# achiever04/face-recognition-platform

Hardware: AMD Instinct MI355X
Metric: faces/sec (detect+embed+match) on 1080p @ 100k gallery (higher is better)
Workload: dtype f16; 1 GPU; 32x1080x1920 BGR frames per GPU per step resident in HBM, host results out every step, 2 batches in flight per GPU (one handle = one stream each, used round-robin), forced K=10 faces/frame, 100000-identity fp16 gallery, FRPDet detector fp16 + ArcFace IResNet-100 fp16 (synthetic seeded weights); batch_frames=32, faces_per_frame=10, gallery=100000, streams=1, lanes=2, lane_warmup_steps=20

## Files before the change

face-recognition-platform_amd/csrc/stem_kernel.hip:

```cpp
#include <hip/hip_runtime.h>
#include <stdint.h>
#include "frp_internal.h"
#include "conv_common.h"

namespace frp {


#define ST_ROWS 4
#define ST_COLS 64
#define ST_PR (2 * ST_ROWS + 1)
#define ST_PE ((2 * ST_COLS + 1) * 3)
#define ST_PITCH 392

__device__ __forceinline__ void bias_relu_pack(const floatx16& acc, int g, floatx4 b, unsigned (&out)[2]) {
#pragma unroll
    for (int h2 = 0; h2 < 2; ++h2) {
        const float2v v = float2v{acc[4 * g + 2 * h2], acc[4 * g + 2 * h2 + 1]} + float2v{b[2 * h2], b[2 * h2 + 1]};
        half2v hv = __builtin_convertvector(v, half2v);
        hv = __builtin_elementwise_max(hv, half2v{0, 0});
        out[h2] = __builtin_bit_cast(unsigned, hv);
    }
}

__device__ __forceinline__ floatx16 mfma16(half8 a, half8 b, floatx16 c) {
    return __builtin_amdgcn_mfma_f32_32x32x16_f16(a, b, c, 0, 0, 0);
}

__global__ __launch_bounds__(256) void stem_u8_kernel(StemParams p) {
    __shared__ __attribute__((aligned(16))) _Float16 patch[ST_PR * ST_PITCH + 16];
    const int t = threadIdx.x, lane = t & 63, wave = t >> 6;
    const int tiles_x = (p.Wo + ST_COLS - 1) / ST_COLS;
    const int tiles_y = (p.Ho + ST_ROWS - 1) / ST_ROWS;
    int bid = blockIdx.x;
    const int tx = bid % tiles_x; bid /= tiles_x;
    const int ty = bid % tiles_y;
    const int b = bid / tiles_y;
    const int oy0 = ty * ST_ROWS, ox0 = tx * ST_COLS;
    const uint8_t* frame = p.frames + (long)b * p.frame_stride;

    const int ix_first = 2 * ox0 - 1;
#pragma unroll
    for (int pr = 0; pr < ST_PR; ++pr) {
        const int iy = 2 * oy0 - 1 + pr;
        const bool yin = (unsigned)iy < (unsigned)p.Hc;
        const bool yimg = (unsigned)iy < (unsigned)p.H;
        const uint8_t* row = frame + (long)(yimg ? iy : 0) * p.row_stride;
        for (int e = t; e < ST_PE; e += 256) {
            const int px = e / 3;
            const int ix = ix_first + px;
            float v = 0.f;
            if (yin && (unsigned)ix < (unsigned)p.Wc) {
                float u = 0.f;
                if (yimg && ix < p.W) u = (float)row[(long)ix * 3 + (e - px * 3)];
                v = (u - 127.5f) * (1.0f / 128.0f);
            }
            const int c = e - px * 3;
            patch[pr * ST_PITCH + px * 3 + (p.rgb_in ? c : 2 - c)] = (_Float16)v;
        }
    }
    for (int e = t; e < ST_PR * (ST_PITCH - ST_PE) + 16; e += 256) {
        if (e < ST_PR * (ST_PITCH - ST_PE)) {
            const int pr = e / (ST_PITCH - ST_PE), off = e - pr * (ST_PITCH - ST_PE);
            patch[pr * ST_PITCH + ST_PE + off] = (_Float16)0.f;
        } else {
            patch[ST_PR * ST_PITCH + (e - ST_PR * (ST_PITCH - ST_PE))] = (_Float16)0.f;
        }
    }

    half8 wa[3];
    {
        const int co = lane & 31, h = lane >> 5;
#pragma unroll
        for (int kh = 0; kh < 3; ++kh)
#pragma unroll
            for (int j = 0; j < 8; ++j) {
                const int k = 8 * h + j;
                _Float16 w = (_Float16)0.f;
                if (k < 9) {
                    const int kw = k / 3, c = k - kw * 3;
                    w = p.w[((co * 3 + kh) * 3 + kw) * 8 + c];
                }
                wa[kh][j] = w;
            }
    }
    __syncthreads();

    const int oy = oy0 + wave;
    const int r = lane & 31, h = lane >> 5;
    const floatx4 bias4[4] = {*reinterpret_cast<const floatx4*>(p.bias + 4 * h), *reinterpret_cast<const floatx4*>(p.bias + 8 + 4 * h),
                              *reinterpret_cast<const floatx4*>(p.bias + 16 + 4 * h), *reinterpret_cast<const floatx4*>(p.bias + 24 + 4 * h)};
#pragma unroll
    for (int half_tile = 0; half_tile < ST_COLS / 32; ++half_tile) {
        const int oxl = half_tile * 32 + r;
        const unsigned* win = reinterpret_cast<const unsigned*>(patch + (2 * wave) * ST_PITCH + 6 * oxl + 8 * h);
        floatx16 acc;
#pragma unroll
        for (int e = 0; e < 16; ++e) acc[e] = 0.f;
#pragma unroll
        for (int kh = 0; kh < 3; ++kh) {
            union { unsigned u[4]; half8 v; } bf;
#pragma unroll
            for (int q = 0; q < 4; ++q) bf.u[q] = win[kh * (ST_PITCH / 2) + q];
            acc = mfma16(wa[kh], bf.v, acc);
        }
        const int ox = ox0 + oxl;
        union { half4 v; unsigned u[2]; } pk[4];
#pragma unroll
        for (int g = 0; g < 4; ++g)
#pragma unroll
            for (int e = 0; e < 4; ++e) pk[g].v[e] = (_Float16)fmaxf(acc[4 * g + e] + bias4[g][e], 0.f);
#pragma unroll
        for (int q = 0; q < 2; ++q) {
            swap_halves(pk[2 * q].u[0], pk[2 * q + 1].u[0]);
            swap_halves(pk[2 * q].u[1], pk[2 * q + 1].u[1]);
        }
        if (oy < p.Ho && ox < p.Wo) {
            _Float16* o = p.out + (((long)b * p.Ho + oy) * p.Wo + ox) * 32;
#pragma unroll
            for (int q = 0; q < 2; ++q)
                *reinterpret_cast<uint4*>(o + 16 * q + 8 * h) = make_uint4(pk[2 * q].u[0], pk[2 * q].u[1], pk[2 * q + 1].u[0], pk[2 * q + 1].u[1]);
        }
    }
}

#define S12_R2 4
#define S12_C2 32
#define S12_S1R (2 * S12_R2 + 1)
#define S12_S1C (2 * S12_C2 + 1)
#define S12_PR (2 * S12_S1R + 1)
#define S12_PE ((2 * S12_S1C + 1) * 3)
#define S12_PITCH 400
#define S12_PATCH_HALFS (S12_PR * S12_PITCH + 16)
#define S12_PIX 80
#define S12_S1BYTES (S12_S1R * 2 * 33 * S12_PIX)

__global__ __launch_bounds__(256, 2) void stem12_u8_kernel(Stem12Params p) {
    __shared__ __attribute__((aligned(16))) _Float16 patch[S12_PATCH_HALFS];
    __shared__ __attribute__((aligned(16))) unsigned char s1[S12_S1BYTES];
    const int t = threadIdx.x, lane = t & 63, wave = t >> 6;
    const int r = lane & 31, h = lane >> 5;
    const int tiles_x = (p.Wo2 + S12_C2 - 1) / S12_C2;
    const int tiles_y = (p.Ho2 + S12_R2 - 1) / S12_R2;
    const int n_tiles = p.B * tiles_y * tiles_x;

    half8 wa[3];
    {
        const int co = r;
#pragma unroll
        for (int kh = 0; kh < 3; ++kh)
#pragma unroll
            for (int j = 0; j < 8; ++j) {
                const int k = 8 * h + j;
                _Float16 w = (_Float16)0.f;
                if (k < 9) {
                    const int kw = k / 3, c = k - kw * 3;
                    w = p.w1[((co * 3 + kh) * 3 + kw) * 8 + 2 - c];
                }
                wa[kh][j] = w;
            }
    }
    const int g2 = wave & 1;
    half8 wb[18];
#pragma unroll
    for (int m = 0; m < 18; ++m)
        wb[m] = *reinterpret_cast<const half8*>(p.w2 + (((g2 * 32 + r) * 9 + (m >> 1)) * 32 + 16 * (m & 1) + 8 * h));
    floatx4 b1[4], b2[4];
#pragma unroll
    for (int g = 0; g < 4; ++g) {
        b1[g] = *reinterpret_cast<const floatx4*>(p.bias1 + 8 * g + 4 * h);
        b2[g] = *reinterpret_cast<const floatx4*>(p.bias2 + 32 * g2 + 8 * g + 4 * h);
    }
    for (int e = t; e < S12_PATCH_HALFS; e += 256) patch[e] = (_Float16)0.f;
    __syncthreads();

    constexpr int DW_ROW = 99;
    constexpr int DW_PER_THREAD = (S12_PR * DW_ROW + 255) / 256;
    const uint8_t* const buf_lo = p.frames;
    const uint8_t* const buf_hi = p.frames + (long)p.B * p.frame_stride;
    unsigned pre[DW_PER_THREAD];
    int rel[DW_PER_THREAD], ldso[DW_PER_THREAD];
#pragma unroll
    for (int i = 0; i < DW_PER_THREAD; ++i) {
        const int idx = t + i * 256;
        const int pr = idx / DW_ROW, d = idx - pr * DW_ROW;
        rel[i] = pr < S12_PR ? pr * (int)p.row_stride + 4 * d : -1;
        ldso[i] = (pr * S12_PITCH + 4 * d) * 2;
    }
    bool pre_fast = false;
    auto tile_interior = [&](int y2_0, int x2_0) {
        const int iy0 = 4 * y2_0 - 3, ix0 = 4 * x2_0 - 3;
        return iy0 >= 0 && iy0 + S12_PR <= p.H && ix0 >= 0 && ix0 + (2 * S12_S1C + 1) + 1 <= p.W;
    };
    auto tile_coords = [&](int tile, int& b, int& y2_0, int& x2_0) {
        int q = tile;
        const int tx = q % tiles_x; q /= tiles_x;
        const int ty = q % tiles_y;
        b = q / tiles_y;
        y2_0 = ty * S12_R2;
        x2_0 = tx * S12_C2;
    };
    auto row_addr = [&](int b, int y2_0, int x2_0, int pr) -> const uint8_t* {
        int iy = 4 * y2_0 - 3 + pr;
        iy = iy < 0 ? 0 : (iy >= p.H ? p.H - 1 : iy);
        return p.frames + (long)b * p.frame_stride + (long)iy * p.row_stride + (long)(4 * x2_0 - 3) * 3;
    };
    auto prefetch = [&](int tile) {
        int b, y2_0, x2_0;
        tile_coords(tile, b, y2_0, x2_0);
        pre_fast = !p.rgb_in && tile_interior(y2_0, x2_0);
        if (pre_fast) {
            const uint8_t* base = p.frames + (long)b * p.frame_stride + (long)(4 * y2_0 - 3) * p.row_stride + (long)(4 * x2_0 - 3) * 3;
#pragma unroll
            for (int i = 0; i < DW_PER_THREAD; ++i) {
                unsigned v = 0u;
                if (rel[i] >= 0) __builtin_memcpy(&v, base + (unsigned)rel[i], 4);
                pre[i] = v;
            }
            return;
        }
#pragma unroll
        for (int i = 0; i < DW_PER_THREAD; ++i) {
            const int idx = t + i * 256;
            const int pr = idx / DW_ROW, d = idx - pr * DW_ROW;
            unsigned v = 0u;
            if (pr < S12_PR) {
                const uint8_t* a = row_addr(b, y2_0, x2_0, pr);
                const uint8_t* al = a - ((uintptr_t)a & 3) + 4 * d;
                if (al >= buf_lo && al + 4 <= buf_hi) {
                    v = *reinterpret_cast<const unsigned*>(al);
                } else {
#pragma unroll
                    for (int j = 0; j < 4; ++j)
                        if (al + j >= buf_lo && al + j < buf_hi) v |= (unsigned)al[j] << (8 * j);
                }
            }
            pre[i] = v;
        }
    };
    if ((int)blockIdx.x < n_tiles) prefetch(blockIdx.x);

    for (int tile = blockIdx.x; tile < n_tiles; tile += gridDim.x) {
        int b, y2_0, x2_0;
        tile_coords(tile, b, y2_0, x2_0);
        const int s1r0 = 2 * y2_0 - 1, s1c0 = 2 * x2_0 - 1;
        const int iy0 = 2 * s1r0 - 1, ix0 = 2 * s1c0 - 1;

        const bool interior = iy0 >= 0 && iy0 + S12_PR <= p.H && ix0 >= 0 && ix0 + (2 * S12_S1C + 1) <= p.W;
        if (pre_fast) {
            const half2v k1024 = {(_Float16)1024.f, (_Float16)1024.f}, kscale = {(_Float16)0.0078125f, (_Float16)0.0078125f},
                         kbias = {(_Float16)-0.99609375f, (_Float16)-0.99609375f};
#pragma unroll
            for (int i = 0; i < DW_PER_THREAD; ++i) {
                if (rel[i] >= 0) {
                    const unsigned lo = __builtin_amdgcn_perm(0x64646464u, pre[i], 0x04010400u);
                    const unsigned hi = __builtin_amdgcn_perm(0x64646464u, pre[i], 0x04030402u);
                    const half2v a = __builtin_elementwise_fma(__builtin_bit_cast(half2v, lo) - k1024, kscale, kbias);
                    const half2v c = __builtin_elementwise_fma(__builtin_bit_cast(half2v, hi) - k1024, kscale, kbias);
                    *reinterpret_cast<uint2*>(reinterpret_cast<unsigned char*>(patch) + ldso[i]) =
                        make_uint2(__builtin_bit_cast(unsigned, a), __builtin_bit_cast(unsigned, c));
                }
            }
        } else {
#pragma unroll
        for (int i = 0; i < DW_PER_THREAD; ++i) {
            const int idx = t + i * 256;
            const int pr = idx / DW_ROW, d = idx - pr * DW_ROW;
            if (pr < S12_PR) {
                const int sh = (int)((uintptr_t)row_addr(b, y2_0, x2_0, pr) & 3);
                const int e0 = 4 * d - sh;
                int px = (e0 + 3) / 3 - 1, c = e0 - px * 3;
                _Float16* prow = patch + pr * S12_PITCH;
                const int iy = iy0 + pr;
                const bool yin = (unsigned)iy < (unsigned)p.Hc;
                const bool yimg = (unsigned)iy < (unsigned)p.H;
#pragma unroll
                for (int j = 0; j < 4; ++j) {
                    const int e = e0 + j;
                    if (e >= 0 && e < S12_PE) {
                        float v = ((float)((pre[i] >> (8 * j)) & 0xffu) - 127.5f) * (1.0f / 128.0f);
                        if (!interior) {
                            const int ix = ix0 + px;
                            const bool in_canvas = yin && (unsigned)ix < (unsigned)p.Wc;
                            const bool in_frame = yimg && ix < p.W;
                            v = in_canvas ? (in_frame ? v : (0.f - 127.5f) * (1.0f / 128.0f)) : 0.f;
                        }
                        prow[px * 3 + (p.rgb_in ? 2 - c : c)] = (_Float16)v;
                    }
                    if (++c == 3) { c = 0; ++px; }
                }
            }
        }
        for (int e = t; e < S12_PR * (S12_PITCH - S12_PE); e += 256) {
            const int pr = e / (S12_PITCH - S12_PE);
            patch[pr * S12_PITCH + S12_PE + (e - pr * (S12_PITCH - S12_PE))] = (_Float16)0.f;
        }
        }
        __syncthreads();
        if (tile + (int)gridDim.x < n_tiles) prefetch(tile + gridDim.x);

        for (int job = wave; job < S12_S1R * 2 + 1; job += 4) {
            const bool extra = job == S12_S1R * 2;
            const int row = extra ? (r < S12_S1R ? r : 0) : job >> 1;
            const int col = extra ? 2 * S12_C2 : (job & 1) * 32 + r;
            const unsigned* win = reinterpret_cast<const unsigned*>(patch + (2 * row) * S12_PITCH + 6 * col + 8 * h);
            floatx16 acc;
#pragma unroll
            for (int e = 0; e < 16; ++e) acc[e] = 0.f;
#pragma unroll
            for (int kh = 0; kh < 3; ++kh) {
                union { unsigned u[4]; half8 v; } bf;
#pragma unroll
                for (int qq = 0; qq < 4; ++qq) bf.u[qq] = win[kh * (S12_PITCH / 2) + qq];
                acc = mfma16(wa[kh], bf.v, acc);
            }
            const int gy = s1r0 + row, gx = s1c0 + col;
            const bool inside = (unsigned)gy < (unsigned)p.Ho1 && (unsigned)gx < (unsigned)p.Wo1;
            struct { unsigned u[2]; } pk[4];
#pragma unroll
            for (int g = 0; g < 4; ++g) {
                bias_relu_pack(acc, g, b1[g], pk[g].u);
                pk[g].u[0] = inside ? pk[g].u[0] : 0u;
                pk[g].u[1] = inside ? pk[g].u[1] : 0u;
            }
#pragma unroll
            for (int qq = 0; qq < 2; ++qq) {
                swap_halves(pk[2 * qq].u[0], pk[2 * qq + 1].u[0]);
                swap_halves(pk[2 * qq].u[1], pk[2 * qq + 1].u[1]);
            }
            if (!extra || r < S12_S1R) {
                unsigned char* dst = s1 + ((row * 2 + (col & 1)) * 33 + (col >> 1)) * S12_PIX;
#pragma unroll
                for (int qq = 0; qq < 2; ++qq)
                    *reinterpret_cast<uint4*>(dst + (2 * qq + h) * 16) =
                        make_uint4(pk[2 * qq].u[0], pk[2 * qq].u[1], pk[2 * qq + 1].u[0], pk[2 * qq + 1].u[1]);
            }
        }
        __syncthreads();

#pragma unroll
        for (int yy = 0; yy < 2; ++yy) {
            const int y = 2 * (wave >> 1) + yy;
            floatx16 acc;
#pragma unroll
            for (int e = 0; e < 16; ++e) acc[e] = 0.f;
#pragma unroll
            for (int m = 0; m < 18; ++m) {
                const int tap = m >> 1, kh = tap / 3, kw = tap - kh * 3;
                const unsigned char* src = s1 + (((2 * y + kh) * 2 + (kw & 1)) * 33 + r + (kw >> 1)) * S12_PIX + (2 * (m & 1) + h) * 16;
                acc = mfma16(wb[m], *reinterpret_cast<const half8*>(src), acc);
            }
            const int oy = y2_0 + y, ox = x2_0 + r;
            struct { unsigned u[2]; } pk[4];
#pragma unroll
            for (int g = 0; g < 4; ++g) bias_relu_pack(acc, g, b2[g], pk[g].u);
#pragma unroll
            for (int qq = 0; qq < 2; ++qq) {
                swap_halves(pk[2 * qq].u[0], pk[2 * qq + 1].u[0]);
                swap_halves(pk[2 * qq].u[1], pk[2 * qq + 1].u[1]);
            }
            if (oy < p.Ho2 && ox < p.Wo2) {
                _Float16* o = p.out + (((long)b * p.Ho2 + oy) * p.Wo2 + ox) * 64 + 32 * g2;
#pragma unroll
                for (int qq = 0; qq < 2; ++qq)
                    *reinterpret_cast<uint4*>(o + 16 * qq + 8 * h) =
                        make_uint4(pk[2 * qq].u[0], pk[2 * qq].u[1], pk[2 * qq + 1].u[0], pk[2 * qq + 1].u[1]);
            }
        }
    }
}

hipError_t launch_stem12_u8(const Stem12Params& p, hipStream_t stream) {
    if (!p.frames || !p.w1 || !p.bias1 || !p.w2 || !p.bias2 || !p.out || p.B <= 0 || p.H <= 0 || p.W <= 0 || p.Hc < p.H ||
        p.Wc < p.W || (p.Hc & 3) || (p.Wc & 3) || p.Ho1 != p.Hc / 2 || p.Wo1 != p.Wc / 2 || p.Ho2 != p.Ho1 / 2 || p.Wo2 != p.Wo1 / 2)
        return hipErrorInvalidValue;
    const long tiles = (long)p.B * ((p.Ho2 + S12_R2 - 1) / S12_R2) * ((p.Wo2 + S12_C2 - 1) / S12_C2);
    if (tiles <= 0 || tiles > 0x7fffffffL) return hipErrorInvalidValue;
    int dev = 0;
    if (hipGetDevice(&dev) != hipSuccess || dev < 0 || dev >= 64) return hipErrorInvalidDevice;
    const int ncu = device_cu_count(dev);
    if (ncu <= 0) return hipErrorInvalidDevice;
    const long slots = 2L * ncu;
    hipLaunchKernelGGL(stem12_u8_kernel, dim3((unsigned)(tiles < slots ? tiles : slots)), dim3(256), 0, stream, p);
    return hipGetLastError();
}

#define ES_ROWS 8
#define ES_COLS 128
#define ES_PITCH 132

__global__ __launch_bounds__(256) void emb_stem_kernel(EmbStemParams p) {
    __shared__ __attribute__((aligned(16))) uint2 patch[(ES_ROWS + 2) * ES_PITCH];
    const int t = threadIdx.x, lane = t & 63, wave = t >> 6;
    const int r = lane & 31, h = lane >> 5;
    const int tiles_x = (p.W + ES_COLS - 1) / ES_COLS;
    const int tiles_y = (p.H + ES_ROWS - 1) / ES_ROWS;
    int q = blockIdx.x;
    const int tx = q % tiles_x; q /= tiles_x;
    const int ty = q % tiles_y;
    const int img = q / tiles_y;
    if (p.n_dev && img >= *p.n_dev) return;
    const int y0 = ty * ES_ROWS, x0 = tx * ES_COLS;
    const _Float16* chip = p.x + (long)img * p.H * p.W * 8;

    for (int e = t; e < (ES_ROWS + 2) * ES_PITCH; e += 256) {
        const int pr = e / ES_PITCH, pc = e - pr * ES_PITCH;
        const int y = y0 - 1 + pr, x = x0 - 1 + pc;
        uint2 v = make_uint2(0u, 0u);
        if ((unsigned)y < (unsigned)p.H && (unsigned)x < (unsigned)p.W)
            v = *reinterpret_cast<const uint2*>(chip + ((long)y * p.W + x) * 8);
        patch[e] = v;
    }
    half8 wa[2][3];
#pragma unroll
    for (int cg = 0; cg < 2; ++cg)
#pragma unroll
        for (int kh = 0; kh < 3; ++kh) {
            const _Float16* w = p.w + (((cg * 32 + r) * 3 + kh) * 3) * 8;
            union { uint2 u[2]; half8 v; } f;
            f.u[0] = *reinterpret_cast<const uint2*>(w + (2 * h) * 8);
            f.u[1] = h ? make_uint2(0u, 0u) : *reinterpret_cast<const uint2*>(w + 8);
            wa[cg][kh] = f.v;
        }
    floatx4 bias[2][4], slope[2][4];
#pragma unroll
    for (int cg = 0; cg < 2; ++cg)
#pragma unroll
        for (int g = 0; g < 4; ++g) {
            bias[cg][g] = *reinterpret_cast<const floatx4*>(p.bias + 32 * cg + 8 * g + 4 * h);
            slope[cg][g] = *reinterpret_cast<const floatx4*>(p.slope + 32 * cg + 8 * g + 4 * h);
        }
    __syncthreads();

#pragma unroll
    for (int yy = 0; yy < 2; ++yy) {
        const int yl = 2 * wave + yy, oy = y0 + yl;
#pragma unroll
        for (int cgp = 0; cgp < ES_COLS / 32; ++cgp) {
            const int xl = cgp * 32 + r, ox = x0 + xl;
            if (x0 + cgp * 32 >= p.W) break;
            floatx16 acc[2];
#pragma unroll
            for (int cg = 0; cg < 2; ++cg)
#pragma unroll
                for (int e = 0; e < 16; ++e) acc[cg][e] = 0.f;
#pragma unroll
            for (int kh = 0; kh < 3; ++kh) {
                const uint2* src = patch + (yl + kh) * ES_PITCH + xl + 2 * h;
                union { uint2 u[2]; half8 v; } bf;
                bf.u[0] = src[0];
                bf.u[1] = src[1];
                acc[0] = mfma16(wa[0][kh], bf.v, acc[0]);
                acc[1] = mfma16(wa[1][kh], bf.v, acc[1]);
            }
#pragma unroll
            for (int cg = 0; cg < 2; ++cg) {
                union { half4 v; unsigned u[2]; } pk[4];
#pragma unroll
                for (int g = 0; g < 4; ++g)
#pragma unroll
                    for (int e = 0; e < 4; ++e) {
                        const float v = acc[cg][4 * g + e] + bias[cg][g][e];
                        pk[g].v[e] = (_Float16)(v > 0.f ? v : v * slope[cg][g][e]);
                    }
#pragma unroll
                for (int qq = 0; qq < 2; ++qq) {
                    swap_halves(pk[2 * qq].u[0], pk[2 * qq + 1].u[0]);
                    swap_halves(pk[2 * qq].u[1], pk[2 * qq + 1].u[1]);
                }
                if (oy < p.H && ox < p.W) {
                    _Float16* o = p.out + (((long)img * p.H + oy) * p.W + ox) * 64 + 32 * cg;
#pragma unroll
                    for (int qq = 0; qq < 2; ++qq)
                        *reinterpret_cast<uint4*>(o + 16 * qq + 8 * h) =
                            make_uint4(pk[2 * qq].u[0], pk[2 * qq].u[1], pk[2 * qq + 1].u[0], pk[2 * qq + 1].u[1]);
                }
            }
        }
    }
}

hipError_t launch_emb_stem(const EmbStemParams& p, hipStream_t stream) {
    if (!p.x || !p.w || !p.bias || !p.slope || !p.out || p.M <= 0 || p.H <= 0 || p.W <= 0) return hipErrorInvalidValue;
    const long tiles = (long)p.M * ((p.H + ES_ROWS - 1) / ES_ROWS) * ((p.W + ES_COLS - 1) / ES_COLS);
    if (tiles <= 0 || tiles > 0x7fffffffL) return hipErrorInvalidValue;
    hipLaunchKernelGGL(emb_stem_kernel, dim3((unsigned)tiles), dim3(256), 0, stream, p);
    return hipGetLastError();
}

hipError_t launch_stem_u8(const StemParams& p, hipStream_t stream) {
    if (!p.frames || !p.w || !p.bias || !p.out || p.B <= 0 || p.H <= 0 || p.W <= 0 || p.Hc < p.H || p.Wc < p.W ||
        (p.Hc & 1) || (p.Wc & 1) || p.Ho != p.Hc / 2 || p.Wo != p.Wc / 2)
        return hipErrorInvalidValue;
    const long tiles = (long)p.B * ((p.Ho + ST_ROWS - 1) / ST_ROWS) * ((p.Wo + ST_COLS - 1) / ST_COLS);
    if (tiles <= 0 || tiles > 0x7fffffffL) return hipErrorInvalidValue;
    hipLaunchKernelGGL(stem_u8_kernel, dim3((unsigned)tiles), dim3(256), 0, stream, p);
    return hipGetLastError();
}

}
```

Baseline: 28160 faces/s.

## Software-pipeline stem12 tile loop: unpack next tile during conv2, batch MFMA jobs

Restructures the persistent stem12 kernel loop so that the next tile's global prefetch is issued right after the first barrier. Its unpack into the LDS patch now runs after the second conv's MFMAs rather than before the next iteration. Stage-1 jobs are processed two at a time with interleaved MFMAs, and stage-2 LDS reads are triple-buffered with sched barriers. The aim is to hide global-load latency and LDS read latency behind MFMA work, at the cost of more registers and explicit vmem waits. Optional FRP_LAB cycle-counter instrumentation is added but compiled out by default.

```diff
diff --git a/face-recognition-platform_amd/csrc/stem_kernel.hip b/face-recognition-platform_amd/csrc/stem_kernel.hip
--- a/face-recognition-platform_amd/csrc/stem_kernel.hip
+++ b/face-recognition-platform_amd/csrc/stem_kernel.hip
@@ -21,6 +21,8 @@
         out[h2] = __builtin_bit_cast(unsigned, hv);
     }
 }
+
+__device__ __forceinline__ void settle_vmem() { __builtin_amdgcn_s_waitcnt(0x0F70); }
 
 __device__ __forceinline__ floatx16 mfma16(half8 a, half8 b, floatx16 c) {
     return __builtin_amdgcn_mfma_f32_32x32x16_f16(a, b, c, 0, 0, 0);
@@ -133,6 +135,17 @@
 #define S12_PATCH_HALFS (S12_PR * S12_PITCH + 16)
 #define S12_PIX 80
 #define S12_S1BYTES (S12_S1R * 2 * 33 * S12_PIX)
+static_assert(S12_S1R * 2 + 1 == 19, "phase B deals jobs w, w + 4, w + 8, w + 12 to wave w and jobs 16 .. 18 to waves 0 .. 2");
+
+#ifdef FRP_LAB
+#define S12_STAMP_WGS 1024
+__device__ unsigned long long g_stem12_stamps[S12_STAMP_WGS * 4 * 8];
+#define S12_CLK(v) const unsigned long long v = __builtin_readcyclecounter()
+#define S12_ADD(acc, a, b) acc += (b) - (a)
+#else
+#define S12_CLK(v)
+#define S12_ADD(acc, a, b)
+#endif
 
 __global__ __launch_bounds__(256, 2) void stem12_u8_kernel(Stem12Params p) {
     __shared__ __attribute__((aligned(16))) _Float16 patch[S12_PATCH_HALFS];
@@ -159,6 +172,7 @@
                 wa[kh][j] = w;
             }
     }
+    const int wave_u = __builtin_amdgcn_readfirstlane(wave);
     const int g2 = wave & 1;
     half8 wb[18];
 #pragma unroll
@@ -204,9 +218,7 @@
         iy = iy < 0 ? 0 : (iy >= p.H ? p.H - 1 : iy);
         return p.frames + (long)b * p.frame_stride + (long)iy * p.row_stride + (long)(4 * x2_0 - 3) * 3;
     };
-    auto prefetch = [&](int tile) {
-        int b, y2_0, x2_0;
-        tile_coords(tile, b, y2_0, x2_0);
+    auto prefetch = [&](int b, int y2_0, int x2_0) {
         pre_fast = !p.rgb_in && tile_interior(y2_0, x2_0);
         if (pre_fast) {
             const uint8_t* base = p.frames + (long)b * p.frame_stride + (long)(4 * y2_0 - 3) * p.row_stride + (long)(4 * x2_0 - 3) * 3;
@@ -237,14 +249,12 @@
             pre[i] = v;
         }
     };
-    if ((int)blockIdx.x < n_tiles) prefetch(blockIdx.x);
-
-    for (int tile = blockIdx.x; tile < n_tiles; tile += gridDim.x) {
-        int b, y2_0, x2_0;
-        tile_coords(tile, b, y2_0, x2_0);
-        const int s1r0 = 2 * y2_0 - 1, s1c0 = 2 * x2_0 - 1;
-        const int iy0 = 2 * s1r0 - 1, ix0 = 2 * s1c0 - 1;
-
+#ifdef FRP_LAB
+    unsigned long long st_a = 0, st_as = 0, st_b1 = 0, st_b = 0, st_b2 = 0, st_c = 0, st_n = 0;
+#endif
+
+    auto unpack = [&](int b, int y2_0, int x2_0) __attribute__((always_inline)) {
+        const int iy0 = 4 * y2_0 - 3, ix0 = 4 * x2_0 - 3;
         const bool interior = iy0 >= 0 && iy0 + S12_PR <= p.H && ix0 >= 0 && ix0 + (2 * S12_S1C + 1) <= p.W;
         if (pre_fast) {
             const half2v k1024 = {(_Float16)1024.f, (_Float16)1024.f}, kscale = {(_Float16)0.0078125f, (_Float16)0.0078125f},
@@ -295,69 +305,134 @@
             patch[pr * S12_PITCH + S12_PE + (e - pr * (S12_PITCH - S12_PE))] = (_Float16)0.f;
         }
         }
+    };
+
+    settle_vmem();
+    int b = 0, y2_0 = 0, x2_0 = 0;
+    if ((int)blockIdx.x < n_tiles) {
+        tile_coords(blockIdx.x, b, y2_0, x2_0);
+        prefetch(b, y2_0, x2_0);
+        unpack(b, y2_0, x2_0);
+        settle_vmem();
+    }
+    S12_CLK(ck_start);
+
+    for (int tile = blockIdx.x; tile < n_tiles; tile += gridDim.x) {
+        const int s1r0 = 2 * y2_0 - 1, s1c0 = 2 * x2_0 - 1;
+        const int next = tile + (int)gridDim.x;
+        S12_CLK(ck1);
         __syncthreads();
-        if (tile + (int)gridDim.x < n_tiles) prefetch(tile + gridDim.x);
-
-        for (int job = wave; job < S12_S1R * 2 + 1; job += 4) {
-            const bool extra = job == S12_S1R * 2;
-            const int row = extra ? (r < S12_S1R ? r : 0) : job >> 1;
-            const int col = extra ? 2 * S12_C2 : (job & 1) * 32 + r;
-            const unsigned* win = reinterpret_cast<const unsigned*>(patch + (2 * row) * S12_PITCH + 6 * col + 8 * h);
-            floatx16 acc;
-#pragma unroll
-            for (int e = 0; e < 16; ++e) acc[e] = 0.f;
-#pragma unroll
-            for (int kh = 0; kh < 3; ++kh) {
-                union { unsigned u[4]; half8 v; } bf;
-#pragma unroll
-                for (int qq = 0; qq < 4; ++qq) bf.u[qq] = win[kh * (S12_PITCH / 2) + qq];
-                acc = mfma16(wa[kh], bf.v, acc);
-            }
-            const int gy = s1r0 + row, gx = s1c0 + col;
-            const bool inside = (unsigned)gy < (unsigned)p.Ho1 && (unsigned)gx < (unsigned)p.Wo1;
+        S12_CLK(ck2);
+        int nb = 0, ny2_0 = 0, nx2_0 = 0;
+        if (next < n_tiles) {
+            tile_coords(next, nb, ny2_0, nx2_0);
+            prefetch(nb, ny2_0, nx2_0);
+        }
+
+        auto stem1_jobs = [&](int job0, int nj) __attribute__((always_inline)) {
+            floatx16 acc[2];
+            union { unsigned u[4]; half8 v; } bf[2][3];
+            int row[2], col[2];
+            bool extra[2];
+#pragma unroll
+            for (int q = 0; q < 2; ++q) {
+                if (q >= nj) break;
+                const int job = job0 + 4 * q;
+                extra[q] = job == S12_S1R * 2;
+                row[q] = extra[q] ? (r < S12_S1R ? r : 0) : job >> 1;
+                col[q] = extra[q] ? 2 * S12_C2 : (job & 1) * 32 + r;
+                const unsigned* win = reinterpret_cast<const unsigned*>(patch + (2 * row[q]) * S12_PITCH + 6 * col[q] + 8 * h);
+#pragma unroll
+                for (int kh = 0; kh < 3; ++kh)
+#pragma unroll
+                    for (int qq = 0; qq < 4; ++qq) bf[q][kh].u[qq] = win[kh * (S12_PITCH / 2) + qq];
+#pragma unroll
+                for (int e = 0; e < 16; ++e) acc[q][e] = 0.f;
+            }
+#pragma unroll
+            for (int kh = 0; kh < 3; ++kh)
+#pragma unroll
+                for (int q = 0; q < 2; ++q) {
+                    if (q >= nj) break;
+                    acc[q] = mfma16(wa[kh], bf[q][kh].v, acc[q]);
+                }
+#pragma unroll
+            for (int q = 0; q < 2; ++q) {
+                if (q >= nj) break;
+                const int gy = s1r0 + row[q], gx = s1c0 + col[q];
+                const bool inside = (unsigned)gy < (unsigned)p.Ho1 && (unsigned)gx < (unsigned)p.Wo1;
+                struct { unsigned u[2]; } pk[4];
+#pragma unroll
+                for (int g = 0; g < 4; ++g) {
+                    bias_relu_pack(acc[q], g, b1[g], pk[g].u);
+                    pk[g].u[0] = inside ? pk[g].u[0] : 0u;
+                    pk[g].u[1] = inside ? pk[g].u[1] : 0u;
+                }
+#pragma unroll
+                for (int qq = 0; qq < 2; ++qq) {
+                    swap_halves(pk[2 * qq].u[0], pk[2 * qq + 1].u[0]);
+                    swap_halves(pk[2 * qq].u[1], pk[2 * qq + 1].u[1]);
+                }
+                if (!extra[q] || r < S12_S1R) {
+                    unsigned char* dst = s1 + ((row[q] * 2 + (col[q] & 1)) * 33 + (col[q] >> 1)) * S12_PIX;
+#pragma unroll
+                    for (int qq = 0; qq < 2; ++qq)
+                        *reinterpret_cast<uint4*>(dst + (2 * qq + h) * 16) =
+                            make_uint4(pk[2 * qq].u[0], pk[2 * qq].u[1], pk[2 * qq + 1].u[0], pk[2 * qq + 1].u[1]);
+                }
+            }
+        };
+        stem1_jobs(wave_u, 2);
+        stem1_jobs(wave_u + 8, 2);
+        if (wave_u < 3) stem1_jobs(wave_u + 16, 1);
+        S12_CLK(ck3);
+        __syncthreads();
+        S12_CLK(ck4);
+
+        floatx16 acc2[2];
+#pragma unroll
+        for (int yy = 0; yy < 2; ++yy)
+#pragma unroll
+            for (int e = 0; e < 16; ++e) acc2[yy][e] = 0.f;
+        {
+            half8 bf[3][2];
+            const unsigned char* s1w = s1 + ((4 * (wave >> 1)) * 2 * 33 + r) * S12_PIX + h * 16;
+            auto rd = [&](int m, int S) {
+                const int tap = m >> 1, kh = tap / 3, kw = tap - kh * 3;
+#pragma unroll
+                for (int yy = 0; yy < 2; ++yy)
+                    bf[S][yy] = *reinterpret_cast<const half8*>(s1w + (((2 * yy + kh) * 2 + (kw & 1)) * 33 + (kw >> 1)) * S12_PIX + (m & 1) * 32);
+            };
+            rd(0, 0);
+            rd(1, 1);
+#pragma unroll
+            for (int m = 0; m < 18; ++m) {
+                if (m + 2 < 18) rd(m + 2, (m + 2) % 3);
+#pragma unroll
+                for (int yy = 0; yy < 2; ++yy) acc2[yy] = mfma16(wb[m], bf[m % 3][yy], acc2[yy]);
+                __builtin_amdgcn_sched_barrier(0);
+            }
+        }
+        S12_CLK(ck5);
+#ifdef FRP_LAB
+        const bool st_fast = pre_fast;
+#endif
+        if (next < n_tiles) unpack(nb, ny2_0, nx2_0);
+        settle_vmem();
+        S12_CLK(ck6);
+#pragma unroll
+        for (int yy = 0; yy < 2; ++yy) {
+            const int y = 2 * (wave >> 1) + yy;
+            const floatx16& acc = acc2[yy];
+            const int oy = y2_0 + y, ox = x2_0 + r;
             struct { unsigned u[2]; } pk[4];
 #pragma unroll
-            for (int g = 0; g < 4; ++g) {
-                bias_relu_pack(acc, g, b1[g], pk[g].u);
-                pk[g].u[0] = inside ? pk[g].u[0] : 0u;
-                pk[g].u[1] = inside ? pk[g].u[1] : 0u;
-            }
+            for (int g = 0; g < 4; ++g) bias_relu_pack(acc, g, b2[g], pk[g].u);
 #pragma unroll
             for (int qq = 0; qq < 2; ++qq) {
                 swap_halves(pk[2 * qq].u[0], pk[2 * qq + 1].u[0]);
                 swap_halves(pk[2 * qq].u[1], pk[2 * qq + 1].u[1]);
             }
-            if (!extra || r < S12_S1R) {
-                unsigned char* dst = s1 + ((row * 2 + (col & 1)) * 33 + (col >> 1)) * S12_PIX;
-#pragma unroll
-                for (int qq = 0; qq < 2; ++qq)
-                    *reinterpret_cast<uint4*>(dst + (2 * qq + h) * 16) =
-                        make_uint4(pk[2 * qq].u[0], pk[2 * qq].u[1], pk[2 * qq + 1].u[0], pk[2 * qq + 1].u[1]);
-            }
-        }
-        __syncthreads();
-
-#pragma unroll
-        for (int yy = 0; yy < 2; ++yy) {
-            const int y = 2 * (wave >> 1) + yy;
-            floatx16 acc;
-#pragma unroll
-            for (int e = 0; e < 16; ++e) acc[e] = 0.f;
-#pragma unroll
-            for (int m = 0; m < 18; ++m) {
-                const int tap = m >> 1, kh = tap / 3, kw = tap - kh * 3;
-                const unsigned char* src = s1 + (((2 * y + kh) * 2 + (kw & 1)) * 33 + r + (kw >> 1)) * S12_PIX + (2 * (m & 1) + h) * 16;
-                acc = mfma16(wb[m], *reinterpret_cast<const half8*>(src), acc);
-            }
-            const int oy = y2_0 + y, ox = x2_0 + r;
-            struct { unsigned u[2]; } pk[4];
-#pragma unroll
-            for (int g = 0; g < 4; ++g) bias_relu_pack(acc, g, b2[g], pk[g].u);
-#pragma unroll
-            for (int qq = 0; qq < 2; ++qq) {
-                swap_halves(pk[2 * qq].u[0], pk[2 * qq + 1].u[0]);
-                swap_halves(pk[2 * qq].u[1], pk[2 * qq + 1].u[1]);
-            }
             if (oy < p.Ho2 && ox < p.Wo2) {
                 _Float16* o = p.out + (((long)b * p.Ho2 + oy) * p.Wo2 + ox) * 64 + 32 * g2;
 #pragma unroll
@@ -366,8 +441,30 @@
                         make_uint4(pk[2 * qq].u[0], pk[2 * qq].u[1], pk[2 * qq + 1].u[0], pk[2 * qq + 1].u[1]);
             }
         }
-    }
-}
+        b = nb; y2_0 = ny2_0; x2_0 = nx2_0;
+#ifdef FRP_LAB
+        S12_CLK(ck7);
+        if (st_fast) S12_ADD(st_a, ck5, ck6); else S12_ADD(st_as, ck5, ck6);
+        S12_ADD(st_b1, ck1, ck2); S12_ADD(st_b, ck2, ck3); S12_ADD(st_b2, ck3, ck4); S12_ADD(st_c, ck4, ck5); S12_ADD(st_c, ck6, ck7);
+        st_n += st_fast ? 1ull : (1ull << 32) + 1ull;
+#endif
+    }
+#ifdef FRP_LAB
+    if (lane == 0 && blockIdx.x < S12_STAMP_WGS) {
+        unsigned long long* o = g_stem12_stamps + ((long)blockIdx.x * 4 + wave) * 8;
+        o[0] = st_a; o[1] = st_as; o[2] = st_b1; o[3] = st_b; o[4] = st_b2; o[5] = st_c; o[6] = st_n;
+        o[7] = __builtin_readcyclecounter() - ck_start;
+    }
+#endif
+}
+
+#ifdef FRP_LAB
+extern "C" __attribute__((visibility("default"))) int frp_lab_stem12_stamps(unsigned long long* out, int n_u64) {
+    if (!out || n_u64 <= 0 || n_u64 > S12_STAMP_WGS * 4 * 8) return -1;
+    if (hipDeviceSynchronize() != hipSuccess) return -2;
+    return hipMemcpyFromSymbol(out, HIP_SYMBOL(g_stem12_stamps), (size_t)n_u64 * 8) == hipSuccess ? 0 : -3;
+}
+#endif
 
 hipError_t launch_stem12_u8(const Stem12Params& p, hipStream_t stream) {
     if (!p.frames || !p.w1 || !p.bias1 || !p.w2 || !p.bias2 || !p.out || p.B <= 0 || p.H <= 0 || p.W <= 0 || p.Hc < p.H ||
```

Result: no change. 28110 faces/s (-0.2%).
